# arclab-hku/ESVIO

Measured on AMD Instinct MI355X. Metric: Mevents/s through time-surface+detect+track @640x480, higher is better.
Workload: dtype f64 timestamps / u8 images / f32 LK sums in the reference build's order

## Files before the change

esvio_amd/csrc/fe_api.cpp:

```cpp
#include "fe_internal.h"

namespace {
typedef int (*nccl_allgather_fn)(const void*, void*, size_t, int , void* ,
                                 hipStream_t);
struct NcclId {
  char internal[128];
};
typedef int (*nccl_get_id_fn)(NcclId*);
typedef int (*nccl_init_rank_fn)(void** , int, NcclId, int);
typedef int (*nccl_destroy_fn)(void*);
void* rccl_lib() {
  static void* lib = []() -> void* {
    const char* names[] = {"librccl.so.1", "librccl.so"};
    for (const char* n : names)
      if (void* l = dlopen(n, RTLD_NOW | RTLD_NOLOAD | RTLD_GLOBAL)) return l;
    for (const char* n : names)
      if (void* l = dlopen(n, RTLD_NOW | RTLD_GLOBAL)) return l;
    return dlopen("/opt/rocm/lib/librccl.so.1", RTLD_NOW | RTLD_GLOBAL);
  }();
  return lib;
}
template <class F>
F rccl_sym(const char* name) {
  void* l = rccl_lib();
// ... 808 lines not shown
  }
  const auto t0 = std::chrono::steady_clock::now();
  while (tap.pending.load(std::memory_order_acquire) > 0 && std::chrono::steady_clock::now() - t0 < std::chrono::seconds(2)) {}
  host::ransac_pool_set_idle_work(pool, nullptr, nullptr, nullptr);
  out3[0] = tap.calls.load();
  out3[1] = tap.done.load();
  out3[2] = (uint64_t)std::max(0, tap.pending.load());
  host::ransac_pool_destroy(pool);
  if (n_inliers) *n_inliers = k;
  return 0;
}

int esvio_fe_lift_projective(const esvio_fe_camera* cam, double u, double v, double* out3) {
  if (!cam || !out3) return ESVIO_FE_EINVAL;
  host::lift_projective(*cam, u, v, out3);
  return 0;
}

static int fill_tracks(esvio_fe_handle c, esvio_fe_tracks* out);
static int track_event_entry(esvio_fe_handle c, double cur_time, const esvio_fe_event* left,
                             size_t nL, const esvio_fe_event* right, size_t nR, int space,
                             int pub_this_frame, const esvio_fe_motion* motion,
                             esvio_fe_tracks* out) {
  if (!c) return ESVIO_FE_EINVAL;
  if (nL == 0 || !left) return fail(c, ESVIO_FE_EINVAL, "left batch must not be empty (node:150)");
  if (nR && !right) return ESVIO_FE_EINVAL;
  if (nL + nR >= (1ull << 31)) return fail(c, ESVIO_FE_EINVAL, "batch too large");
  HIPCHK(c, hipSetDevice(c->dev));
  if (int rc = track_event_impl(c, cur_time, left, nL, right, nR, space, pub_this_frame != 0, motion))
    return rc;
// ... 3560 lines not shown
```

esvio_amd/csrc/fe_ctx.h:

```cpp
#pragma once
#include <hip/hip_runtime.h>

#include <algorithm>
#include <atomic>
#include <chrono>
#include <cmath>
#include <cstdarg>
#include <cstdio>
#include <cstdlib>
#include <cstring>
#include <dlfcn.h>
#include <map>
#include <string>
#include <utility>
#include <deque>
#include <vector>

#include "../../include/esvio_fe.h"
#include "../../include/esvio_fe_test.h"
#include "fe_aedat.h"
#include "fe_bag.h"
#include "fe_host.h"
#include "fe_kernels.h"
#include "fe_layout.h"
// ... 13 lines not shown
  void build(const std::vector<int>& ids, const std::vector<P2f>& pts) {
    v.clear();
    v.reserve(ids.size());
    for (size_t i = 0; i < ids.size(); i++) v.emplace_back(ids[i], pts[i]);
    std::stable_sort(v.begin(), v.end(),
                     [](const std::pair<int, P2f>& a, const std::pair<int, P2f>& b) { return a.first < b.first; });
    v.erase(std::unique(v.begin(), v.end(),
                        [](const std::pair<int, P2f>& a, const std::pair<int, P2f>& b) { return a.first == b.first; }),
            v.end());
  }
  const P2f* find(int id) const {
    auto it = std::lower_bound(v.begin(), v.end(), id,
                               [](const std::pair<int, P2f>& a, int k) { return a.first < k; });
    return (it != v.end() && it->first == id) ? &it->second : nullptr;
  }
};

const char* const kKernelNames[K_COUNT] = {
    "k_tile_hist", "k_tile_scan", "k_tile_scatter", "k_tile_apply", "k_sae_keys", "k_radix_pass", "k_sae_apply",
    "k_time_surface4", "k_time_surface", "k_median", "k_clahe", "k_norm_pyr", "k_pyr3", "k_pyr_down", "k_pyr_pad",
    "k_scharr", "k_pad_scharr", "k_lk_f32", "k_lk", "k_arc_map", "k_arc_ev", "k_dedup", "k_compact", "k_select_mw",
    "k_select", "k_select_gbm", "k_fast_score", "k_fast_collect", "k_events_from_fields", "k_baf_heads", "k_baf_filter",
    "k_baf_count", "k_baf_scan", "k_baf_emit", "k_baf_keys_fields", "k_baf_emit_fields", "k_raw_reduce", "k_raw_scan",
    "k_raw_emit", "k_slice_reduce", "k_slice_scan", "k_slice_cuts", "k_baf_keys_addr", "k_hot_count", "k_hot_keys",
    "k_hot_pick", "k_trig_reduce", "k_trig_emit"};
const char* const kIngestKernelNames[K_INGEST_COUNT - K_COUNT] = {"k_aedat_count", "k_aedat_scan", "k_aedat_emit", "k_bag_emit", "k_image_emit"};

enum Phase {
  PH_ENQ_BATCH, PH_ENQ_TEMPORAL, PH_WAIT_TEMPORAL, PH_FILTER, PH_RANSAC, PH_MASK_DETECT, PH_WAIT_STEREO, PH_TAIL,
  PH_PUB_SETMASK, PH_PUB_SELECT, PH_PUB_SPEC, PH_PUB_PREV_RIGHT, PH_PUB_STEREO_NEW, PH_PUB_PREFETCH,
// ... 446 lines not shown
    DevBuf<uint2> kids;
    DevBuf<int32_t> node_word;
    DevBuf<double> node_weight, word_weight;
    DevBuf<uint32_t> desc, keys[2], vals[2], sort, heads, q_word, cnt;
    DevBuf<int32_t> word, err;
    DevBuf<double> weight, q_val;
    uint32_t q_n = 0;
    DevBuf<uint32_t> db_word;
    DevBuf<double> db_val;
    DevBuf<uint64_t> db_off;
    std::vector<uint64_t> off = std::vector<uint64_t>(1, 0);
    DevBuf<double> score, res_score, res_raw;
    DevBuf<uint8_t> present;
    DevBuf<int32_t> res_id;
  } bow;
};

namespace esvio {
namespace fe {

inline thread_local hipStream_t t_stream_override = nullptr;
inline hipStream_t stereo_stream(const esvio_fe_ctx* c) { return c->stereo_unpub ? c->stream6 : c->stream4; }
inline hipStream_t cur_stream(const esvio_fe_ctx* c) {
  return t_stream_override ? t_stream_override : c->stream;
}
struct StreamScope {
  hipStream_t saved;
  explicit StreamScope(hipStream_t s) : saved(t_stream_override) { t_stream_override = s; }
  ~StreamScope() { t_stream_override = saved; }
};
// ... 96 lines not shown
```

esvio_amd/csrc/fe_host.cpp:

```cpp
#include "fe_host.h"

#include <algorithm>
#include <cfloat>
#include <climits>
#include <cmath>
#include <cstdio>
#include <cstdlib>
#include <cstring>

#include <atomic>
#include <chrono>
#include <condition_variable>
#include <sys/resource.h>
#include <memory>
#include <mutex>
#include <thread>

#if defined(__linux__)
#include <pthread.h>
#include <sched.h>
#endif

#if defined(__HIP_DEVICE_COMPILE__) || defined(ESVIO_NO_SIMD_CLONES)
#define ESVIO_SIMD_CLONES
#else
#define ESVIO_SIMD_CLONES __attribute__((target_clones("avx512f", "avx2", "default")))
#endif

namespace esvio {
namespace host {

int cv_round(double v) {
  if (!(v > -2147483648.5 && v < 2147483647.5)) return INT_MIN;
  const double r = std::nearbyint(v);
  if (r > 2147483647.0 || r < -2147483648.0) return INT_MIN;
  return (int)r;
}

int cv_floor(float v) {
  int i = (int)v;
  return i - (i > v);
}

static void radtan(const esvio_fe_camera& c, double x, double y, double& dx, double& dy) {
  const double x2 = x * x, y2 = y * y, xy = x * y;
  const double rho2 = x2 + y2;
  const double rad = c.k1 * rho2 + c.k2 * rho2 * rho2;
// ... 1353 lines not shown
```

esvio_amd/csrc/fe_host.h:

```cpp
#pragma once
#include <atomic>
#include <stdint.h>

#include <vector>

#include "../../include/esvio_fe.h"
#include "../../include/esvio_fe_test.h"

namespace esvio {
inline void cpu_relax() {
#if !defined(__HIP_DEVICE_COMPILE__) && (defined(__x86_64__) || defined(__i386__))
  __builtin_ia32_pause();
#endif
}
namespace host {

int cv_round(double v);
int cv_floor(float v);

void lift_projective(const esvio_fe_camera& cam, double u, double v, double out[3]);
void lift_projective_batch(const esvio_fe_camera& cam, const float* uv, int n, double* xu, double* yu);

std::vector<int> disc_halfwidths(int r);

struct BitMask {
  int W = 0, H = 0, wpr = 0;
  std::vector<uint32_t> bits;
  void reset(int w, int h);
  bool test(int x, int y) const { return (bits[(size_t)y * wpr + (x >> 5)] >> (x & 31)) & 1u; }
  void stamp_disc(int cx, int cy, int r, const std::vector<int>& hw);
  void from_bytes(const uint8_t* mask);
};
// ... 20 lines not shown
```

esvio_amd/csrc/fe_internal.h:

```cpp
#pragma once
#include "fe_ctx.h"

namespace esvio {
namespace fe {

template <class T>
void reduce_vector(std::vector<T>& v, const std::vector<uint8_t>& status) {
  int j = 0;
  for (int i = 0; i < int(v.size()); i++)
    if (status[i]) v[j++] = v[i];
  v.resize(j);
}

inline uint8_t* px00(const PyrDesc& d) { return d.img[0] + (size_t)kPad * d.stride[0] + kPad; }

inline int lookback_expired(esvio_fe_ctx* c) {
  return c->pin[0].counts[3] ? fail(c, ESVIO_FE_EINTERNAL, "radix sort look-back spin expired") : 0;
}

int ensure_event_capacity(esvio_fe_ctx* c, size_t n);
int ensure_sort_capacity(esvio_fe_ctx* c, size_t n);
int ensure_part_capacity(esvio_fe_ctx* c, size_t n, bool mc);
int ensure_cand_capacity(esvio_fe_ctx* c, int set, size_t n);
int ensure_arc_capacity(esvio_fe_ctx* c, size_t n, int set);
// ... 31 lines not shown
               int flags);
void run_lk(esvio_fe_ctx* c, const LkArgs& f, const LkArgs* b, float2* back_pts, uint8_t* back_status);
enum LkPairKind { kLkTemporal, kLkStereo };
struct LkPair {
  LkArgs f, b;
  LkOut out;
};
LkPair lk_pair(const PyrDesc& P, const PyrDesc& N, const P2f* src, const int* n_ptr, int n_max, LkPairKind kind,
               const LkOut& out);
void run_lk_pair(esvio_fe_ctx* c, const LkPair& p);
int copy_level0_out(esvio_fe_ctx* c, const PyrDesc& d, uint8_t* out);
int copy_level0_in(esvio_fe_ctx* c, const PyrDesc& d, const uint8_t* in, int space = ESVIO_FE_HOST);
bool in_border_event(const esvio_fe_ctx* c, const P2f& pt);
double pt_distance(const P2f& a, const P2f& b);
void event_set_mask(esvio_fe_ctx* c);
std::vector<P2f> undistorted_pts(const std::vector<P2f>& pts, const esvio_fe_camera& cam);
std::vector<P2f> pts_velocity_fn(std::vector<int>& ids, std::vector<P2f>& pts, IdMap& cur_id_pts,
                                 IdMap& prev_id_pts, double dt, size_t n_left);
void reject_with_f_event(esvio_fe_ctx* c);
void clear_tracker_state(esvio_fe_ctx* c);
SelectArgs make_select_args(esvio_fe_ctx* c, int set, int max_corners, float2* out_pts, int out_base,
                            int32_t* out_idx);
size_t select_lds_bytes(const esvio_fe_ctx* c);
KernelId launch_select_args(esvio_fe_ctx* c, SelectArgs s);
void compact_set(esvio_fe_ctx* c, const esvio_fe_ctx::CandSet& cs, uint32_t nblk, bool booked);
void run_select(esvio_fe_ctx* c, int set, int max_corners, float2* out_pts, int out_base, int32_t* out_idx,
                const uint32_t* mask_bits = nullptr, int* host_counts = nullptr, bool publish = false,
                const float2* stamp_pts = nullptr, int n_stamp = 0);
void run_arc(esvio_fe_ctx* c, const EventRec* ev, uint32_t n, const PyrDesc* ts, bool use_mask,
             bool want_flags, bool want_cand, int set, bool marked = false);
// ... 58 lines not shown
```

esvio_amd/csrc/fe_stages.cpp:

```cpp
#include "fe_internal.h"

#include <optional>

namespace esvio {
namespace fe {


int ensure_event_capacity(esvio_fe_ctx* c, size_t n) { return c->d_ev.grow(c, n); }

static int grow_sort_buffers(esvio_fe_ctx* c, size_t cap) {
  c->sort_cap = 0;
  for (int i = 0; i < 2; i++) {
    c->keys[i].release();
    c->vals[i].release();
  }
  for (int i = 0; i < 2; i++) {
    if (int rc = c->keys[i].alloc(c, cap)) return rc;
    if (int rc = c->vals[i].alloc(c, cap)) return rc;
  }
  if (int rc = c->sae_marks.alloc(c, cap)) return rc;
  c->sort_cap = cap;
  return 0;
}

// ... 481 lines not shown
}


bool in_border_event(const esvio_fe_ctx* c, const P2f& pt) {
  const int BORDER_SIZE = 1;
  const int img_x = host::cv_round(pt.x), img_y = host::cv_round(pt.y);
  return BORDER_SIZE <= img_x && img_x < c->W - BORDER_SIZE && BORDER_SIZE <= img_y &&
         img_y < c->H - BORDER_SIZE;
}

double pt_distance(const P2f& a, const P2f& b) {
  const double dx = a.x - b.x, dy = a.y - b.y;
  return std::sqrt(dx * dx + dy * dy);
}

void event_set_mask(esvio_fe_ctx* c) {
  c->mask_event.reset(c->W, c->H);
  struct Item {
    int first;
    std::pair<P2f, int> second;
    int src;
  };
  std::vector<Item> cnt_pts_id;
  cnt_pts_id.reserve(c->cur_pts.size());
  for (unsigned int i = 0; i < c->cur_pts.size(); i++)
    cnt_pts_id.push_back(Item{c->track_cnt[i], std::make_pair(c->cur_pts[i], c->ids[i]), c->src_idx[i]});
  std::sort(cnt_pts_id.begin(), cnt_pts_id.end(),
            [](const Item& a, const Item& b) { return a.first > b.first; });
  c->cur_pts.clear();
  c->ids.clear();
  c->track_cnt.clear();
  c->src_idx.clear();
  for (auto& it : cnt_pts_id) {
    const int px = host::cv_round(it.second.first.x), py = host::cv_round(it.second.first.y);
    if (px < 0 || px >= c->W || py < 0 || py >= c->H) continue;
    if (!c->mask_event.test(px, py)) {
      c->cur_pts.push_back(it.second.first);
      c->ids.push_back(it.second.second);
      c->track_cnt.push_back(it.first);
      c->src_idx.push_back(it.src);
      c->mask_event.stamp_disc(px, py, c->cfg.min_dist, c->hw);
    }
  }
}

std::vector<P2f> undistorted_pts(const std::vector<P2f>& pts, const esvio_fe_camera& cam) {
  const size_t n = pts.size();
  std::vector<P2f> un(n);
  if (!n) return un;
  std::vector<double> lx(n), ly(n);
  host::lift_projective_batch(cam, &pts[0].x, (int)n, lx.data(), ly.data());
  for (size_t i = 0; i < n; i++) un[i] = P2f{(float)lx[i], (float)ly[i]};
  return un;
}

std::vector<P2f> pts_velocity_fn(std::vector<int>& ids, std::vector<P2f>& pts, IdMap& cur_id_pts,
                                 IdMap& prev_id_pts, double dt, size_t n_left) {
  std::vector<P2f> vel;
// ... 10 lines not shown
        vel.push_back(P2f{0, 0});
      }
    }
  } else {
    vel.assign(n_left, P2f{0, 0});
  }
  return vel;
}

void reject_with_f_event(esvio_fe_ctx* c) {
  if (c->trace) c->tr_fm_class[c->cur_pts.size() < 8 ? 0 : c->cur_pts.size() < 15 ? 1 : 2]++;
  if (c->cur_pts.size() >= 8) {
    const esvio_fe_camera& cam = c->cfg.cam[0];
    const double FOCAL = c->cfg.focal_length;
    const size_t n = c->prev_pts.size();
    std::vector<float> un_cur(n * 2), un_prev(n * 2);
    std::vector<double> lx(n), ly(n);
    const double cx = c->W / 2.0, cy = c->H / 2.0;
    const auto tl = std::chrono::steady_clock::now();
    const bool pre = c->pre_lift_valid && c->pre_lx.size() == n;
    if (!pre) host::lift_projective_batch(cam, &c->prev_pts[0].x, (int)n, lx.data(), ly.data());
    const double* plx = pre ? c->pre_lx.data() : lx.data();
    const double* ply = pre ? c->pre_ly.data() : ly.data();
    c->pre_lift_valid = false;
    for (size_t i = 0; i < n; i++) {
      un_prev[2 * i] = (float)(FOCAL * plx[i] / 1.0 + cx);
      un_prev[2 * i + 1] = (float)(FOCAL * ply[i] / 1.0 + cy);
    }
    host::lift_projective_batch(cam, &c->cur_pts[0].x, (int)n, lx.data(), ly.data());
    for (size_t i = 0; i < n; i++) {
      un_cur[2 * i] = (float)(FOCAL * lx[i] / 1.0 + cx);
      un_cur[2 * i + 1] = (float)(FOCAL * ly[i] / 1.0 + cy);
    }
    std::vector<uint8_t> status(c->cur_pts.size());
    const auto t0 = std::chrono::steady_clock::now();
    host::find_fundamental_mat(un_prev.data(), un_cur.data(), (int)c->cur_pts.size(),
                               c->cfg.f_threshold, 0.99, status.data(), c->pool);
    if (c->trace) {
      const double ms = std::chrono::duration<double, std::milli>(std::chrono::steady_clock::now() - t0).count();
      c->tr_fm_ms += ms;
      c->tr_fm_max_ms = std::max(c->tr_fm_max_ms, ms);
      c->tr_lift_ms += std::chrono::duration<double, std::milli>(t0 - tl).count();
    }
    reduce_vector(c->prev_pts, status);
    reduce_vector(c->cur_pts, status);
    reduce_vector(c->ids, status);
    reduce_vector(c->track_cnt, status);
    reduce_vector(c->src_idx, status);
  }
// ... 166 lines not shown
```

esvio_amd/csrc/fe_track.cpp:

```cpp
#include "fe_internal.h"

#include <sched.h>
#include <sys/resource.h>

#include <atomic>
#include <condition_variable>
#include <mutex>
#include <thread>

namespace esvio {
namespace fe {

struct PrefetchJob {
  Inflight b;
  bool wait_planes = false;
  int lks_wait = -1;
};

static int prefetch_issue(esvio_fe_ctx* c, const PrefetchJob& j) {
  const Inflight& b = j.b;
  StreamScope on_prefetch_stream(c->stream2);
  PrefetchBatchScope its_event_images(&b);
  if (j.wait_planes) HIPCHK(c, hipStreamWaitEvent(c->stream2, c->ev_planes_free, 0));
  if (j.lks_wait >= 0) HIPCHK(c, hipStreamWaitEvent(c->stream2, c->ev_lks_done[j.lks_wait], 0));
  const EventRec *dL = b.dL, *dR = b.dR;
  if (b.stage >= 0) {
    if (int rc = stager_attach(c, b.stage, b.nL, c->stream2, &dL, &dR)) return rc;
  } else if (int rc = stage_events(c, b.left, b.nL, b.right, b.nR, b.space, &dL, &dR, b.lane)) {
    return rc;
  }
  bool arc_marked = false;
  McParams mcp;
// ... 46 lines not shown
        if ((++spins & 1023) == 0 &&
            std::chrono::steady_clock::now() - idle_since > std::chrono::microseconds(2000)) {
          std::unique_lock<std::mutex> lk(mu);
          sleeping.store(true, std::memory_order_seq_cst);
          cv.wait(lk, [&] {
            return submitted.load(std::memory_order_seq_cst) != done.load(std::memory_order_relaxed) ||
                   quit.load(std::memory_order_seq_cst);
          });
          sleeping.store(false, std::memory_order_seq_cst);
          idle_since = std::chrono::steady_clock::now();
        }
        continue;
      }
      const PrefetchJob& job = ring[d % kRing];
      if (first_rc.load(std::memory_order_relaxed) == 0) {
        const int rc = prefetch_issue(c, job);
        if (rc) first_rc.store(rc, std::memory_order_release);
      }
      if (first_rc.load(std::memory_order_relaxed) != 0 && job.b.gate) {
        launch_set_u32(c->stream2, c->d_lane_gate + job.b.lane, job.b.gate);
        (void)hipGetLastError();
      }
      done.store(d + 1, std::memory_order_release);
      idle_since = std::chrono::steady_clock::now();
    }
  }
};

int stereo_split_prepare(esvio_fe_ctx* c) {
  if (c->stream6) return 0;
  const bool wanted = c->stereo_split_env >= 0 ? c->stereo_split_env != 0 : (c->cfg.lk_accum == 2 && c->launcher != nullptr);
  if (!wanted) return 0;
  HIPCHK(c, c->stream6.create());
  launch_spin(c->stream6, 0);
  HIPCHK(c, hipStreamSynchronize(c->stream6));
  return 0;
}

int launcher_set(esvio_fe_ctx* c, bool on) {
  if (on == (c->launcher != nullptr)) return 0;
  if (on) {
    for (uint64_t& j : c->lane_job) j = 0;
    c->lks_wait_job[0] = c->lks_wait_job[1] = 0;
    Launcher* l = new Launcher();
    l->c = c;
    l->th = std::thread([l] { l->run(); });
    c->launcher = l;
    return 0;
  }
  const int rc = launcher_drain(c);
  if (rc && !c->launch_err) c->launch_err = rc;
  for (uint64_t& j : c->lane_job) j = 0;
  c->lks_wait_job[0] = c->lks_wait_job[1] = 0;
  Launcher* l = c->launcher;
  l->quit.store(true, std::memory_order_seq_cst);
  { std::lock_guard<std::mutex> g(l->mu); }
  l->cv.notify_all();
  l->th.join();
  delete l;
  c->launcher = nullptr;
  return rc;
}

static int launcher_result(esvio_fe_ctx* c) {
  const int rc = c->launcher->first_rc.load(std::memory_order_acquire);
  if (rc) c->err = c->launcher->err_text.empty() ? "a prefetch job of the launch thread failed" : c->launcher->err_text;
  return rc;
}

void launcher_clear_error(esvio_fe_ctx* c) {
  if (c->launcher) c->launcher->first_rc.store(0, std::memory_order_release);
  c->launch_err = 0;
}

int launcher_drain(esvio_fe_ctx* c) {
  Launcher* l = c->launcher;
  if (!l) return 0;
  while (l->done.load(std::memory_order_acquire) != l->submitted.load(std::memory_order_relaxed)) cpu_relax();
  return launcher_result(c);
}

int launcher_wait_lane(esvio_fe_ctx* c, int lane) {
  Launcher* l = c->launcher;
  if (!l) return 0;
  while (l->done.load(std::memory_order_acquire) < c->lane_job[lane]) cpu_relax();
  return launcher_result(c);
}

int record_lks_done(esvio_fe_ctx* c, int set) {
  if (Launcher* l = c->launcher) {
    while (l->done.load(std::memory_order_acquire) < c->lks_wait_job[set]) cpu_relax();
    if (int rc = launcher_result(c)) return rc;
  }
  HIPCHK(c, hipEventRecord(c->ev_lks_done[set], stereo_stream(c)));
  c->lks_last = set;
  return 0;
}

static int launcher_submit(esvio_fe_ctx* c, const PrefetchJob& j) {
  Launcher* l = c->launcher;
  const uint64_t s = l->submitted.load(std::memory_order_relaxed);
  l->ring[s % Launcher::kRing] = j;
  c->lane_job[j.b.lane] = s + 1;
  if (j.lks_wait >= 0) c->lks_wait_job[j.lks_wait] = s + 1;
  l->submitted.store(s + 1, std::memory_order_seq_cst);
  if (l->sleeping.load(std::memory_order_seq_cst)) {
    { std::lock_guard<std::mutex> g(l->mu); }
    l->cv.notify_all();
  }
  return 0;
}

int prefetch_next(esvio_fe_ctx* c, bool wait_planes, bool must_take_first) {
  int rc = 0;
  const bool only_first = must_take_first;
  const bool async_ok = c->launcher && !c->prof_on && !c->trace && !must_take_first;
  if (c->launcher && !async_ok)
    if ((rc = launcher_drain(c))) return rc;
  while (!rc && !c->announced.empty() && (int)c->inflight.size() < kPrefetchDepth) {
    PrefetchJob job;
    Inflight& b = job.b;
    static_cast<Batch&>(b) = c->announced.front();
    if (b.stage >= 0 && !must_take_first && !stager_ready(c, b.stage)) break;
    must_take_first = false;
// ... 92 lines not shown
  if (c->chain_enabled && c->waits_fit_chain && !nxt.pub && c->inflight.size() >= 2 && c->inflight[0].lane == nxt.lane &&
      !c->chain_valid)
    nxt2 = &c->inflight[1];
  if (nxt2) {
    sp.f.chain_out = c->d_chain;
    sp.f.chain_seq = next_chain_seq(c);
  }
  {
    StreamScope on_spec_stream(c->stream3);
    run_lk_pair(c, sp);
  }
  HIPCHK(c, hipEventRecord(c->ev_spec_done, c->stream3));
  c->spec_valid = true;
  if (nxt2) {
    const bool gated = c->launcher && nxt2->gate != 0;
    if (!gated)
      if (int rc = launcher_wait_lane(c, nxt2->lane)) return rc;
    HIPCHK(c, hipStreamWaitEvent(c->stream4, c->ev_lane_done[nxt.lane], 0));
    if (!gated) HIPCHK(c, hipStreamWaitEvent(c->stream4, c->ev_lane_done[nxt2->lane], 0));
    const PyrDesc& N2 = c->pyr[nxt2->slotL].d;
    LkPair ch = lk_pair(N, N2, nullptr, nullptr, n_max, kLkTemporal, c->zspec[1].out);
    ch.f.chain_in = c->d_chain;
    ch.f.chain_seq = c->chain_seq;
    ch.f.chain_ticks = c->lim.chain;
    ch.f.poll_err = c->zspec[1].expired;
    if (gated) {
      ch.f.gate_ptr = c->d_lane_gate + nxt2->lane;
      ch.f.gate_val = nxt2->gate;
    }
    {
// ... 2 lines not shown
    }
    HIPCHK(c, hipEventRecord(c->ev_chain_done, c->stream4));
    c->chain_valid = true;
    c->tr_chain_launch++;
    c->chain_for = c->frame_no + 2;
    c->chain_map_ok = false;
  }
  return 0;
}

int cancel_chain(esvio_fe_ctx* c) {
  if (!c->chain_valid) return 0;
  c->chain_valid = false;
  c->chain_map_ok = false;
  c->tr_chain_cancel++;
  HIPCHK(c, hipStreamSynchronize(c->stream4));
  return 0;
}

void right_tail(esvio_fe_ctx* c, const LkOut& kept, const P2f* left, const int* ids, const int* src,
                int n, int n_kept, double dt, size_t n_left) {
  const esvio_fe_config& cfg = c->cfg;
  c->ids_right.clear();
  c->cur_right_pts.clear();
  c->cur_un_right_pts.clear();
  c->right_pts_velocity.clear();
  c->cur_un_right_pts_map.clear();
  c->track_cnt_right.clear();
  if (n_left) {
    std::vector<uint8_t> status(n), statusRightLeft(n);
// ... 343 lines not shown
    c->pre_lift_valid = false;
    const PyrDesc& prevL = c->pyr[c->slot_prevL].d;
    const PyrDesc& curL = c->pyr[c->slot_curL].d;
    if (c->prev_pts.size() > 0) {
      const int n = (int)c->prev_pts.size();
      LkOut t{};
      bool spec_ok = false;
      if (use_spec) {
        if (int rc = await_early(c->ev_spec_done, 0, &spec_ok)) return rc;
        t = c->hspec[0].out;
        if (!spec_ok) {
          c->n_spec_expired++;
          HIPCHK(c, hipStreamSynchronize(c->stream3));
        }
      }
      std::vector<P2f> g_ptsB, g_ptsC;
      std::vector<uint8_t> g_stA, g_stB;
      if (use_chain) {
        if (int rc = await_early(c->ev_chain_done, 1, &spec_ok)) return rc;
        c->tr_chain_used += spec_ok;
        if (!spec_ok) c->n_chain_expired++;
        if (c->trace && spec_ok) trace_chain_intervals();
        if (spec_ok) {
          const LkOut& r = c->hspec[1].out;
          g_ptsB.resize(n);
          g_ptsC.resize(n);
          g_stA.resize(n);
          g_stB.resize(n);
          for (int j = 0; j < n; j++) {
            const int k = c->chain_map[j];
            g_ptsB[j] = r.fwd[k];
            g_ptsC[j] = r.back[k];
// ... 22 lines not shown
          st.f.chain_ticks = c->lim.chain;
          st.f.poll_err = c->zspec[1].expired;
          StreamScope on_stereo_stream(stereo_stream(c));
          HIPCHK(c, hipStreamWaitEvent(stereo_stream(c), c->ev_imgs_ready, 0));
          run_lk_pair(c, st);
          if (int rc = record_lks_done(c, c->res_set)) return rc;
        }
        if (int rc = early_work()) return rc;
        if (int rc = exchange_flush(c)) return rc;
        pre_lift();
        lap(PH_ENQ_TEMPORAL);
        HIPCHK(c, sync_main(c));
        lap(PH_WAIT_TEMPORAL);
        t = pin.s1;
      }
      std::vector<uint8_t> status(t.st_fwd, t.st_fwd + n);
      c->cur_pts.resize(n);
      std::memcpy(c->cur_pts.data(), t.fwd, (size_t)n * 8);
      if (cfg.flow_back) {
        const P2f* reverse_pts = t.back;
        for (int i = 0; i < n; i++) {
          if (status[i] && t.st_back[i] && pt_distance(c->prev_pts[i], reverse_pts[i]) <= 0.5)
            status[i] = 1;
          else
            status[i] = 0;
        }
      }
      for (int i = 0; i < n; i++)
        if (status[i] && !in_border_event(c, c->cur_pts[i])) status[i] = 0;
      if (chain_covers_next) {
        if (use_spec && spec_ok) {
// ... 59 lines not shown
    const PyrDesc& curR = c->pyr[c->slot_curR].d;
    n_surv = (int)c->cur_pts.size();
    c->src_idx.resize(n_surv);
    for (int i = 0; i < n_surv; i++) c->src_idx[i] = stereo_chained ? surv_src[i] : i;
    lap(PH_FILTER);
    n_kept = n_surv;
    will_spec = (have_next || had_announced) && c->waits_fit_spec;
    if (!PUB_THIS_FRAME) {
      if (int rc = upload_kept()) return rc;
      if (will_spec && n_kept && !c->chain_valid)
        if (const Inflight* nb = next_batch())
          if (int rc = enqueue_spec_temporal(c, *nb, n_kept, false)) return rc;
    }
    if (n_surv && !stereo_chained) {
      std::memcpy(pin.A, c->cur_pts.data(), (size_t)n_surv * 8);
      {
        StreamScope on_stereo_stream(stereo_stream(c));
        run_lk_pair(c, lk_pair(curL, curR, zpin.A, nullptr, n_surv, kLkStereo, zpin.s1));
        if (int rc = record_lks_done(c, c->res_set)) return rc;
      }
    }
    return 0;
  }

  int publish() {
    const esvio_fe_config& cfg = c->cfg;
    const PyrDesc& curL = c->pyr[c->slot_curL].d;
    const PyrDesc& curR = c->pyr[c->slot_curR].d;
    if (PUB_THIS_FRAME) {
      if (cfg.f_ransac) reject_with_f_event(c);
      lap(PH_RANSAC);
      PhaseClock parts;
      auto sub = [&](Phase p) { c->lat.cur_phase[p] += parts.lap(); };
// ... 61 lines not shown
        c->cur_pts.push_back(p);
        c->ids.push_back(c->n_id++);
        c->track_cnt.push_back(1);
      }
    }
    const int pub = PUB_THIS_FRAME ? 1 : 0;
    PhaseClock tt;
    auto tail_lap = [&](int i) { if (c->trace) c->tail_ms[pub][i] += tt.lap(); };
    c->cur_un_pts = undistorted_pts(c->cur_pts, cfg.cam[0]);
    c->pts_velocity = pts_velocity_fn(c->ids, c->cur_un_pts, c->cur_un_pts_map, c->prev_un_pts_map,
                                      c->cur_time - c->prev_time, c->cur_pts.size());
    lap(PH_TAIL);
    tail_lap(0);
    const bool lazy = c->lazy_new && detect;
    const bool defer_right = c->lazy_new && !PUB_THIS_FRAME;
    bool pending_later = false;
    if (defer_right && c->pend.active && !c->pend_right.active) {
      pending_later = c->lazy_late || !event_over(c->ev_lknew_done);
    }
    if (!pending_later)
      if (int rc = finalize_lazy(c)) return rc;
    tail_lap(1);
    if (defer_right) {
    } else {
      if (!lazy) HIPCHK(c, sync_main(c));
      if (n_surv || stereo_chained) HIPCHK(c, sync_event(c->ev_lks_done[c->res_set]));
      if (stereo_chained) {
        if (take_expired(1)) {
          c->n_chain_expired++;
          const int n = (int)surv_src.size() ? surv_src.back() + 1 : 0;
          if (n) {
            const PyrDesc& curL = c->pyr[c->slot_curL].d;
            const PyrDesc& curR = c->pyr[c->slot_curR].d;
            StreamScope on_stereo_stream(stereo_stream(c));
            run_lk_pair(c, lk_pair(curL, curR, zpin.s1.fwd, nullptr, n, kLkStereo, c->zpin[set_st].s1));
            HIPCHK(c, hipStreamSynchronize(stereo_stream(c)));
          }
        }
      }
    }
// ... 120 lines not shown
  c->stereo_unpub = !PUB_THIS_FRAME && c->stereo_split;
  c->frame_no++;
  t.pin = c->pin[c->res_set];
  t.zpin = c->zpin[c->res_set];
  if (PUB_THIS_FRAME && c->pool) host::ransac_pool_wake(c->pool);
  c->cur_time = _cur_time;
  c->lat.cur_phase[PH_CHECK] = t.clock.lap();
  int rc = t.take_batch();
  if (!rc) {
    t.lap(PH_ENQ_BATCH);
    rc = t.temporal();
  }
  if (!rc) rc = t.survivors_stereo();
  if (!rc) rc = t.publish();
  if (!rc) rc = t.tails();
  if (rc && c->cur_stage >= 0) {
    (void)launcher_drain(c);
    (void)hipStreamSynchronize(c->stream);
    (void)hipStreamSynchronize(c->stream2);
    (void)hipStreamSynchronize(c->stream4);
    if (c->stream6) (void)hipStreamSynchronize(c->stream6);
    (void)hipGetLastError();
    stager_abandon(c, c->cur_stage);
    c->cur_stage = -1;
  }
  if (!rc) latency_commit(c, PUB_THIS_FRAME, t0, cpu0, sw0, allocs0);
  return rc;
}


// ... 3 lines not shown
```

esvio_amd/frontend.py:

```python
import ctypes as C
import os

import numpy as np

from . import build as _build

_HERE = os.path.dirname(os.path.abspath(__file__))
HOST, DEVICE = 0, 1
EVENT_IMAGES_AHEAD = 2
LK_USE_INITIAL_FLOW = 4


class FrontendError(RuntimeError):
    pass


class Camera(C.Structure):
    _fields_ = [(n, C.c_double) for n in ("fx", "fy", "cx", "cy", "k1", "k2", "p1", "p2")]


class Config(C.Structure):
    _fields_ = [
        ("width", C.c_int32), ("height", C.c_int32),
        ("decay_ms", C.c_double),
# ... 282 lines not shown
    "esvio_fe_track_image", "esvio_fe_unregister_host_buffer", "esvio_fe_version",
    "esvio_fe_kf_set_pattern", "esvio_fe_kf_blur", "esvio_fe_kf_fast", "esvio_fe_kf_brief", "esvio_fe_kf_match",
    "esvio_fe_kf_describe",
    "esvio_fe_bow_vocabulary_header", "esvio_fe_bow_set_vocabulary", "esvio_fe_bow_transform", "esvio_fe_bow_add",
    "esvio_fe_bow_query", "esvio_fe_bow_detect_loop", "esvio_fe_bow_clear", "esvio_fe_bow_entries", "esvio_fe_bow_reserve",
]
TEST_SYMBOLS = [
    "esvio_fe_build_pyramid", "esvio_fe_debug_counters", "esvio_fe_debug_inject", "esvio_fe_device_memory",
    "esvio_fe_export_level",
    "esvio_fe_find_fundamental_mat_held", "esvio_fe_find_fundamental_mat_idle", "esvio_fe_find_fundamental_mat_mt",
    "esvio_fe_get_kernel_stats", "esvio_fe_host_hypot", "esvio_fe_host_nullspace", "esvio_fe_host_stage_copy",
    "esvio_fe_host_stage_pack", "esvio_fe_staging_counters",
    "esvio_fe_kernel_count", "esvio_fe_kernel_name", "esvio_fe_latency_phase_name", "esvio_fe_latency_recent",
    "esvio_fe_latency_stats", "esvio_fe_lift_projective", "esvio_fe_plain_call_counters", "esvio_fe_ransac_stats",
    "esvio_fe_ransac_tail", "esvio_fe_raw_tile_bytes", "esvio_fe_reset_kernel_stats", "esvio_fe_select_candidates",
    "esvio_fe_set_profiling", "esvio_fe_set_sae",
    "esvio_fe_slice_tile_events", "esvio_fe_stage_kernel_count", "esvio_fe_stream",
    "esvio_fe_aedat_tile_events", "esvio_fe_ingest_kernel_count", "esvio_fe_aedat_walk_tap", "esvio_fe_aedat_walk_state_bytes",
    "esvio_fe_bag_tile_events", "esvio_fe_bag_walk_tap", "esvio_fe_bag_walk_state_bytes",
    "esvio_fe_bag_image_walk_tap", "esvio_fe_image_tile_pixels", "esvio_fe_event_image_kernel_stats",
    "esvio_fe_aedat_frame_walk_tap", "esvio_fe_aedat_frame_kernel_stats", "esvio_fe_frame16_tile_pixels",
    "esvio_fe_kf_kernel_count", "esvio_fe_kf_kernel_name", "esvio_fe_kf_kernel_stats", "esvio_fe_kf_blur_tile",
    "esvio_fe_bow_kernel_count", "esvio_fe_bow_kernel_name", "esvio_fe_bow_kernel_stats", "esvio_fe_bow_limits", "esvio_fe_bow_scores",
]

LATENCY_PHASES = 16
SELECT_EUCLID, SELECT_TABLE = 1, 2


class LatencyCall(C.Structure):
    _fields_ = [("call", C.c_uint64), ("published", C.c_int32), ("reserved", C.c_int32), ("begin_ms", C.c_double),
# ... 1763 lines not shown
    rc = L.esvio_fe_lift_projective(C.byref(c), float(u), float(v), _p(out))
    if rc:
        raise FrontendError("lift_projective rc=%d" % rc)
    return out


def aedat_header(data):
    buf = bytes(data)
    info = AedatHeaderInfo()
    rc = load_library().esvio_fe_aedat_header(buf if buf else None, len(buf), C.byref(info))
    if rc:
        raise FrontendError("esvio_fe_aedat_header rc=%d" % rc)
    return info


def aedat_walk_tap(state, data, runs_cap=None, events_cap=None):
    L = load_library()
    nst = L.esvio_fe_aedat_walk_state_bytes()
    st = np.zeros(nst, np.uint8) if state is None else np.frombuffer(bytes(state), np.uint8).copy()
    buf = np.frombuffer(bytes(data), np.uint8)
    events_cap = buf.nbytes // 8 + 1 if events_cap is None else events_cap
    runs_cap = events_cap if runs_cap is None else runs_cap
    runs, pay, counts = np.zeros((max(runs_cap, 1), 2), np.uint32), np.zeros(max(events_cap, 1) * 8, np.uint8), np.zeros(4, np.uint64)
    rc = L.esvio_fe_aedat_walk_tap(_p(st), nst, _p(buf) if buf.nbytes else None, buf.nbytes, _p(runs), runs_cap, _p(pay), events_cap, _p(counts))
    if rc:
        raise FrontendError("esvio_fe_aedat_walk_tap rc=%d" % rc)
    n, nr = int(counts[0]), int(counts[1])
    r = np.stack([runs[:nr, 0].astype(np.int64), runs[:nr, 1].view(np.int32).astype(np.int64)], axis=1) if nr else np.zeros((0, 2), np.int64)
    return st.tobytes(), r, pay[:8 * n].tobytes(), tuple(int(v) for v in counts)

# ... 77 lines not shown
```

Measured before the change: 2943.

## Cut host overhead: SIMD set_mask, inline cvRound, scratch reuse, async stereo LK launch

Replaces the bitmap-stamping set_mask with a pairwise check against kept points, using SSE2 to reject candidates eight at a time, and makes cv_round an inline SSE2 conversion. Per-frame vectors in reject/filter are moved into reusable context scratch to avoid allocations. The stereo LK launch is handed to the launcher thread on publish frames, with waits added before dependent syncs. It also drops a pending-later event check and adds a test tap; these add synchronization complexity and could change rounding or behavior in edge cases.

```diff
diff --git a/esvio_amd/csrc/fe_api.cpp b/esvio_amd/csrc/fe_api.cpp
--- a/esvio_amd/csrc/fe_api.cpp
+++ b/esvio_amd/csrc/fe_api.cpp
@@ -846,6 +846,35 @@
 int esvio_fe_lift_projective(const esvio_fe_camera* cam, double u, double v, double* out3) {
   if (!cam || !out3) return ESVIO_FE_EINVAL;
   host::lift_projective(*cam, u, v, out3);
+  return 0;
+}
+
+int esvio_fe_set_mask_tap(int width, int height, int min_dist, int form, const float* xy, const int32_t* ids,
+                          const int32_t* track_cnt, int n, float* out_xy, int32_t* out_ids, int32_t* out_cnt,
+                          int32_t* out_src, int32_t* n_out) {
+  if (width <= 0 || height <= 0 || min_dist < 1 || min_dist > kMaxDiscR || (form != 0 && form != 1) || n < 0 || !n_out)
+    return ESVIO_FE_EINVAL;
+  if (n && (!xy || !ids || !track_cnt || !out_xy || !out_ids || !out_cnt || !out_src)) return ESVIO_FE_EINVAL;
+  std::vector<P2f> pts(n);
+  std::vector<int> id(n), cnt(n), src(n);
+  for (int i = 0; i < n; i++) {
+    pts[i] = P2f{xy[2 * i], xy[2 * i + 1]};
+    id[i] = ids[i];
+    cnt[i] = track_cnt[i];
+    src[i] = i;
+  }
+  SetMaskScratch scratch;
+  host::BitMask bitmap;
+  set_mask_points(width, height, min_dist, host::disc_halfwidths(min_dist), pts, id, cnt, src, scratch,
+                  form ? &bitmap : nullptr);
+  for (size_t k = 0; k < pts.size(); k++) {
+    out_xy[2 * k] = pts[k].x;
+    out_xy[2 * k + 1] = pts[k].y;
+    out_ids[k] = id[k];
+    out_cnt[k] = cnt[k];
+    out_src[k] = src[k];
+  }
+  *n_out = (int32_t)pts.size();
   return 0;
 }
 
diff --git a/esvio_amd/csrc/fe_ctx.h b/esvio_amd/csrc/fe_ctx.h
--- a/esvio_amd/csrc/fe_ctx.h
+++ b/esvio_amd/csrc/fe_ctx.h
@@ -51,6 +51,21 @@
                                [](const std::pair<int, P2f>& a, int k) { return a.first < k; });
     return (it != v.end() && it->first == id) ? &it->second : nullptr;
   }
+};
+
+struct SetMaskItem {
+  int first;
+  std::pair<P2f, int> second;
+  int src;
+};
+struct SetMaskScratch {
+  std::vector<SetMaskItem> items;
+  std::vector<int16_t> kx, ky;
+};
+struct RejectScratch {
+  std::vector<float> un_cur, un_prev;
+  std::vector<double> lx, ly;
+  std::vector<uint8_t> status;
 };
 
 const char* const kKernelNames[K_COUNT] = {
@@ -527,6 +542,14 @@
     DevBuf<uint8_t> present;
     DevBuf<int32_t> res_id;
   } bow;
+
+  SetMaskScratch set_mask_scratch;
+  RejectScratch reject_scratch;
+  struct FilterScratch {
+    std::vector<uint8_t> status, stA, stB;
+    std::vector<P2f> ptsB, ptsC;
+  } filter_scratch;
+  uint64_t stereo_job = 0;
 };
 
 namespace esvio {
diff --git a/esvio_amd/csrc/fe_host.cpp b/esvio_amd/csrc/fe_host.cpp
--- a/esvio_amd/csrc/fe_host.cpp
+++ b/esvio_amd/csrc/fe_host.cpp
@@ -30,7 +30,7 @@
 namespace esvio {
 namespace host {
 
-int cv_round(double v) {
+int cv_round_portable(double v) {
   if (!(v > -2147483648.5 && v < 2147483647.5)) return INT_MIN;
   const double r = std::nearbyint(v);
   if (r > 2147483647.0 || r < -2147483648.0) return INT_MIN;
diff --git a/esvio_amd/csrc/fe_host.h b/esvio_amd/csrc/fe_host.h
--- a/esvio_amd/csrc/fe_host.h
+++ b/esvio_amd/csrc/fe_host.h
@@ -7,6 +7,11 @@
 #include "../../include/esvio_fe.h"
 #include "../../include/esvio_fe_test.h"
 
+#if !defined(__HIP_DEVICE_COMPILE__) && defined(__x86_64__)
+#include <emmintrin.h>
+#define ESVIO_HOST_SSE2 1
+#endif
+
 namespace esvio {
 inline void cpu_relax() {
 #if !defined(__HIP_DEVICE_COMPILE__) && (defined(__x86_64__) || defined(__i386__))
@@ -15,7 +20,14 @@
 }
 namespace host {
 
-int cv_round(double v);
+int cv_round_portable(double v);
+inline int cv_round(double v) {
+#ifdef ESVIO_HOST_SSE2
+  return _mm_cvtsd_si32(_mm_set_sd(v));
+#else
+  return cv_round_portable(v);
+#endif
+}
 int cv_floor(float v);
 
 void lift_projective(const esvio_fe_camera& cam, double u, double v, double out[3]);
diff --git a/esvio_amd/csrc/fe_internal.h b/esvio_amd/csrc/fe_internal.h
--- a/esvio_amd/csrc/fe_internal.h
+++ b/esvio_amd/csrc/fe_internal.h
@@ -69,6 +69,8 @@
 bool in_border_event(const esvio_fe_ctx* c, const P2f& pt);
 double pt_distance(const P2f& a, const P2f& b);
 void event_set_mask(esvio_fe_ctx* c);
+void set_mask_points(int W, int H, int r, const std::vector<int>& hw, std::vector<P2f>& pts, std::vector<int>& ids,
+                     std::vector<int>& track_cnt, std::vector<int>& src_idx, SetMaskScratch& s, host::BitMask* bitmap);
 std::vector<P2f> undistorted_pts(const std::vector<P2f>& pts, const esvio_fe_camera& cam);
 std::vector<P2f> pts_velocity_fn(std::vector<int>& ids, std::vector<P2f>& pts, IdMap& cur_id_pts,
                                  IdMap& prev_id_pts, double dt, size_t n_left);
diff --git a/esvio_amd/csrc/fe_stages.cpp b/esvio_amd/csrc/fe_stages.cpp
--- a/esvio_amd/csrc/fe_stages.cpp
+++ b/esvio_amd/csrc/fe_stages.cpp
@@ -1,6 +1,11 @@
 #include "fe_internal.h"
 
 #include <optional>
+
+#if !defined(__HIP_DEVICE_COMPILE__) && defined(__x86_64__)
+#include <emmintrin.h>
+#define ESVIO_SET_MASK_SSE2 1
+#endif
 
 namespace esvio {
 namespace fe {
@@ -519,34 +524,76 @@
   return std::sqrt(dx * dx + dy * dy);
 }
 
-void event_set_mask(esvio_fe_ctx* c) {
-  c->mask_event.reset(c->W, c->H);
-  struct Item {
-    int first;
-    std::pair<P2f, int> second;
-    int src;
+static bool in_kept_disc(const int16_t* kx, const int16_t* ky, int nk, int px, int py, int r, const int* hw) {
+  auto exact = [&](int j) {
+    const int dy = std::abs(py - ky[j]), dx = std::abs(px - kx[j]);
+    return dy <= r && dx <= hw[dy];
   };
-  std::vector<Item> cnt_pts_id;
-  cnt_pts_id.reserve(c->cur_pts.size());
-  for (unsigned int i = 0; i < c->cur_pts.size(); i++)
-    cnt_pts_id.push_back(Item{c->track_cnt[i], std::make_pair(c->cur_pts[i], c->ids[i]), c->src_idx[i]});
+  int j = 0;
+#ifdef ESVIO_SET_MASK_SSE2
+  const __m128i vx = _mm_set1_epi16((short)(px + r)), vy = _mm_set1_epi16((short)(py + r));
+  const __m128i lim = _mm_set1_epi16((short)(2 * r)), zero = _mm_setzero_si128();
+  for (; j + 8 <= nk; j += 8) {
+    const __m128i ex = _mm_subs_epu16(_mm_sub_epi16(vx, _mm_loadu_si128((const __m128i*)(kx + j))), lim);
+    const __m128i ey = _mm_subs_epu16(_mm_sub_epi16(vy, _mm_loadu_si128((const __m128i*)(ky + j))), lim);
+    int m = _mm_movemask_epi8(_mm_cmpeq_epi16(_mm_or_si128(ex, ey), zero));
+    for (; m; m &= m - 1) {
+      const int bit = __builtin_ctz((unsigned)m);
+      if (!(bit & 1) && exact(j + (bit >> 1))) return true;
+    }
+  }
+#endif
+  for (; j < nk; j++)
+    if (exact(j)) return true;
+  return false;
+}
+
+void set_mask_points(int W, int H, int r, const std::vector<int>& hw, std::vector<P2f>& pts, std::vector<int>& ids,
+                     std::vector<int>& track_cnt, std::vector<int>& src_idx, SetMaskScratch& s, host::BitMask* bitmap) {
+  if (bitmap) bitmap->reset(W, H);
+  using Item = SetMaskItem;
+  std::vector<Item>& cnt_pts_id = s.items;
+  cnt_pts_id.clear();
+  cnt_pts_id.reserve(pts.size());
+  for (unsigned int i = 0; i < pts.size(); i++)
+    cnt_pts_id.push_back(Item{track_cnt[i], std::make_pair(pts[i], ids[i]), src_idx[i]});
   std::sort(cnt_pts_id.begin(), cnt_pts_id.end(),
             [](const Item& a, const Item& b) { return a.first > b.first; });
-  c->cur_pts.clear();
-  c->ids.clear();
-  c->track_cnt.clear();
-  c->src_idx.clear();
+  pts.clear();
+  ids.clear();
+  track_cnt.clear();
+  src_idx.clear();
+  s.kx.resize(cnt_pts_id.size());
+  s.ky.resize(cnt_pts_id.size());
+  int nk = 0;
+  const bool pairwise = !bitmap && W <= 16384 && H <= 16384 && r <= 255;
+  host::BitMask own;
+  if (!bitmap && !pairwise) {
+    own.reset(W, H);
+    bitmap = &own;
+  }
   for (auto& it : cnt_pts_id) {
     const int px = host::cv_round(it.second.first.x), py = host::cv_round(it.second.first.y);
-    if (px < 0 || px >= c->W || py < 0 || py >= c->H) continue;
-    if (!c->mask_event.test(px, py)) {
-      c->cur_pts.push_back(it.second.first);
-      c->ids.push_back(it.second.second);
-      c->track_cnt.push_back(it.first);
-      c->src_idx.push_back(it.src);
-      c->mask_event.stamp_disc(px, py, c->cfg.min_dist, c->hw);
+    if (px < 0 || px >= W || py < 0 || py >= H) continue;
+    if (bitmap ? !bitmap->test(px, py) : !in_kept_disc(s.kx.data(), s.ky.data(), nk, px, py, r, hw.data())) {
+      pts.push_back(it.second.first);
+      ids.push_back(it.second.second);
+      track_cnt.push_back(it.first);
+      src_idx.push_back(it.src);
+      if (bitmap) {
+        bitmap->stamp_disc(px, py, r, hw);
+      } else {
+        s.kx[nk] = (int16_t)px;
+        s.ky[nk] = (int16_t)py;
+        nk++;
+      }
     }
   }
+}
+
+void event_set_mask(esvio_fe_ctx* c) {
+  set_mask_points(c->W, c->H, c->cfg.min_dist, c->hw, c->cur_pts, c->ids, c->track_cnt, c->src_idx, c->set_mask_scratch,
+                  nullptr);
 }
 
 std::vector<P2f> undistorted_pts(const std::vector<P2f>& pts, const esvio_fe_camera& cam) {
@@ -587,8 +634,13 @@
     const esvio_fe_camera& cam = c->cfg.cam[0];
     const double FOCAL = c->cfg.focal_length;
     const size_t n = c->prev_pts.size();
-    std::vector<float> un_cur(n * 2), un_prev(n * 2);
-    std::vector<double> lx(n), ly(n);
+    RejectScratch& s = c->reject_scratch;
+    std::vector<float>&un_cur = s.un_cur, &un_prev = s.un_prev;
+    std::vector<double>&lx = s.lx, &ly = s.ly;
+    un_cur.resize(n * 2);
+    un_prev.resize(n * 2);
+    lx.resize(n);
+    ly.resize(n);
     const double cx = c->W / 2.0, cy = c->H / 2.0;
     const auto tl = std::chrono::steady_clock::now();
     const bool pre = c->pre_lift_valid && c->pre_lx.size() == n;
@@ -605,7 +657,8 @@
       un_cur[2 * i] = (float)(FOCAL * lx[i] / 1.0 + cx);
       un_cur[2 * i + 1] = (float)(FOCAL * ly[i] / 1.0 + cy);
     }
-    std::vector<uint8_t> status(c->cur_pts.size());
+    std::vector<uint8_t>& status = s.status;
+    status.assign(c->cur_pts.size(), 0);
     const auto t0 = std::chrono::steady_clock::now();
     host::find_fundamental_mat(un_prev.data(), un_cur.data(), (int)c->cur_pts.size(),
                                c->cfg.f_threshold, 0.99, status.data(), c->pool);
diff --git a/esvio_amd/csrc/fe_track.cpp b/esvio_amd/csrc/fe_track.cpp
--- a/esvio_amd/csrc/fe_track.cpp
+++ b/esvio_amd/csrc/fe_track.cpp
@@ -15,7 +15,18 @@
   Inflight b;
   bool wait_planes = false;
   int lks_wait = -1;
+  bool stereo = false;
+  LkPair lk{};
+  hipStream_t stream = nullptr;
+  int lks_set = 0;
 };
+
+static int stereo_issue(esvio_fe_ctx* c, const PrefetchJob& j) {
+  StreamScope on_stereo_stream(j.stream);
+  run_lk_pair(c, j.lk);
+  HIPCHK(c, hipEventRecord(c->ev_lks_done[j.lks_set], j.stream));
+  return 0;
+}
 
 static int prefetch_issue(esvio_fe_ctx* c, const PrefetchJob& j) {
   const Inflight& b = j.b;
@@ -92,7 +103,7 @@
       }
       const PrefetchJob& job = ring[d % kRing];
       if (first_rc.load(std::memory_order_relaxed) == 0) {
-        const int rc = prefetch_issue(c, job);
+        const int rc = job.stereo ? stereo_issue(c, job) : prefetch_issue(c, job);
         if (rc) first_rc.store(rc, std::memory_order_release);
       }
       if (first_rc.load(std::memory_order_relaxed) != 0 && job.b.gate) {
@@ -120,6 +131,7 @@
   if (on) {
     for (uint64_t& j : c->lane_job) j = 0;
     c->lks_wait_job[0] = c->lks_wait_job[1] = 0;
+    c->stereo_job = 0;
     Launcher* l = new Launcher();
     l->c = c;
     l->th = std::thread([l] { l->run(); });
@@ -130,6 +142,7 @@
   if (rc && !c->launch_err) c->launch_err = rc;
   for (uint64_t& j : c->lane_job) j = 0;
   c->lks_wait_job[0] = c->lks_wait_job[1] = 0;
+  c->stereo_job = 0;
   Launcher* l = c->launcher;
   l->quit.store(true, std::memory_order_seq_cst);
   { std::lock_guard<std::mutex> g(l->mu); }
@@ -158,6 +171,15 @@
   return launcher_result(c);
 }
 
+static int launcher_wait_stereo(esvio_fe_ctx* c) {
+  if (!c->stereo_job) return 0;
+  const uint64_t job = std::exchange(c->stereo_job, 0);
+  Launcher* l = c->launcher;
+  if (!l) return 0;
+  while (l->done.load(std::memory_order_acquire) < job) cpu_relax();
+  return launcher_result(c);
+}
+
 int launcher_wait_lane(esvio_fe_ctx* c, int lane) {
   Launcher* l = c->launcher;
   if (!l) return 0;
@@ -166,6 +188,7 @@
 }
 
 int record_lks_done(esvio_fe_ctx* c, int set) {
+  if (int rc = launcher_wait_stereo(c)) return rc;
   if (Launcher* l = c->launcher) {
     while (l->done.load(std::memory_order_acquire) < c->lks_wait_job[set]) cpu_relax();
     if (int rc = launcher_result(c)) return rc;
@@ -173,6 +196,14 @@
   HIPCHK(c, hipEventRecord(c->ev_lks_done[set], stereo_stream(c)));
   c->lks_last = set;
   return 0;
+}
+
+static void launcher_publish(Launcher* l, uint64_t s) {
+  l->submitted.store(s + 1, std::memory_order_seq_cst);
+  if (l->sleeping.load(std::memory_order_seq_cst)) {
+    { std::lock_guard<std::mutex> g(l->mu); }
+    l->cv.notify_all();
+  }
 }
 
 static int launcher_submit(esvio_fe_ctx* c, const PrefetchJob& j) {
@@ -181,11 +212,23 @@
   l->ring[s % Launcher::kRing] = j;
   c->lane_job[j.b.lane] = s + 1;
   if (j.lks_wait >= 0) c->lks_wait_job[j.lks_wait] = s + 1;
-  l->submitted.store(s + 1, std::memory_order_seq_cst);
-  if (l->sleeping.load(std::memory_order_seq_cst)) {
-    { std::lock_guard<std::mutex> g(l->mu); }
-    l->cv.notify_all();
-  }
+  launcher_publish(l, s);
+  return 0;
+}
+
+static int launcher_submit_stereo(esvio_fe_ctx* c, const LkPair& lk, hipStream_t stream, int set) {
+  if (int rc = launcher_wait_stereo(c)) return rc;
+  Launcher* l = c->launcher;
+  const uint64_t s = l->submitted.load(std::memory_order_relaxed);
+  PrefetchJob& j = l->ring[s % Launcher::kRing];
+  j.stereo = true;
+  j.b.gate = 0;
+  j.lk = lk;
+  j.stream = stream;
+  j.lks_set = set;
+  c->stereo_job = s + 1;
+  c->lks_last = set;
+  launcher_publish(l, s);
   return 0;
 }
 
@@ -308,6 +351,7 @@
   c->spec_valid = true;
   if (nxt2) {
     const bool gated = c->launcher && nxt2->gate != 0;
+    if (int rc = launcher_wait_stereo(c)) return rc;
     if (!gated)
       if (int rc = launcher_wait_lane(c, nxt2->lane)) return rc;
     HIPCHK(c, hipStreamWaitEvent(c->stream4, c->ev_lane_done[nxt.lane], 0));
@@ -340,6 +384,7 @@
   c->chain_valid = false;
   c->chain_map_ok = false;
   c->tr_chain_cancel++;
+  if (int rc = launcher_wait_stereo(c)) return rc;
   HIPCHK(c, hipStreamSynchronize(c->stream4));
   return 0;
 }
@@ -713,8 +758,8 @@
           HIPCHK(c, hipStreamSynchronize(c->stream3));
         }
       }
-      std::vector<P2f> g_ptsB, g_ptsC;
-      std::vector<uint8_t> g_stA, g_stB;
+      std::vector<P2f>&g_ptsB = c->filter_scratch.ptsB, &g_ptsC = c->filter_scratch.ptsC;
+      std::vector<uint8_t>&g_stA = c->filter_scratch.stA, &g_stB = c->filter_scratch.stB;
       if (use_chain) {
         if (int rc = await_early(c->ev_chain_done, 1, &spec_ok)) return rc;
         c->tr_chain_used += spec_ok;
@@ -767,7 +812,8 @@
         lap(PH_WAIT_TEMPORAL);
         t = pin.s1;
       }
-      std::vector<uint8_t> status(t.st_fwd, t.st_fwd + n);
+      std::vector<uint8_t>& status = c->filter_scratch.status;
+      status.assign(t.st_fwd, t.st_fwd + n);
       c->cur_pts.resize(n);
       std::memcpy(c->cur_pts.data(), t.fwd, (size_t)n * 8);
       if (cfg.flow_back) {
@@ -857,9 +903,12 @@
     }
     if (n_surv && !stereo_chained) {
       std::memcpy(pin.A, c->cur_pts.data(), (size_t)n_surv * 8);
-      {
+      const LkPair st = lk_pair(curL, curR, zpin.A, nullptr, n_surv, kLkStereo, zpin.s1);
+      if (PUB_THIS_FRAME && c->launcher && !c->prof_on && !c->trace) {
+        if (int rc = launcher_submit_stereo(c, st, stereo_stream(c), c->res_set)) return rc;
+      } else {
         StreamScope on_stereo_stream(stereo_stream(c));
-        run_lk_pair(c, lk_pair(curL, curR, zpin.A, nullptr, n_surv, kLkStereo, zpin.s1));
+        run_lk_pair(c, st);
         if (int rc = record_lks_done(c, c->res_set)) return rc;
       }
     }
@@ -951,16 +1000,14 @@
     tail_lap(0);
     const bool lazy = c->lazy_new && detect;
     const bool defer_right = c->lazy_new && !PUB_THIS_FRAME;
-    bool pending_later = false;
-    if (defer_right && c->pend.active && !c->pend_right.active) {
-      pending_later = c->lazy_late || !event_over(c->ev_lknew_done);
-    }
+    const bool pending_later = defer_right && c->pend.active && !c->pend_right.active;
     if (!pending_later)
       if (int rc = finalize_lazy(c)) return rc;
     tail_lap(1);
     if (defer_right) {
     } else {
       if (!lazy) HIPCHK(c, sync_main(c));
+      if (int rc = launcher_wait_stereo(c)) return rc;
       if (n_surv || stereo_chained) HIPCHK(c, sync_event(c->ev_lks_done[c->res_set]));
       if (stereo_chained) {
         if (take_expired(1)) {
@@ -1111,6 +1158,8 @@
   if (!rc) rc = t.survivors_stereo();
   if (!rc) rc = t.publish();
   if (!rc) rc = t.tails();
+  if (int rc2 = launcher_wait_stereo(c))
+    if (!rc) rc = rc2;
   if (rc && c->cur_stage >= 0) {
     (void)launcher_drain(c);
     (void)hipStreamSynchronize(c->stream);
diff --git a/esvio_amd/frontend.py b/esvio_amd/frontend.py
--- a/esvio_amd/frontend.py
+++ b/esvio_amd/frontend.py
@@ -320,7 +320,7 @@
     "esvio_fe_kernel_count", "esvio_fe_kernel_name", "esvio_fe_latency_phase_name", "esvio_fe_latency_recent",
     "esvio_fe_latency_stats", "esvio_fe_lift_projective", "esvio_fe_plain_call_counters", "esvio_fe_ransac_stats",
     "esvio_fe_ransac_tail", "esvio_fe_raw_tile_bytes", "esvio_fe_reset_kernel_stats", "esvio_fe_select_candidates",
-    "esvio_fe_set_profiling", "esvio_fe_set_sae",
+    "esvio_fe_set_mask_tap", "esvio_fe_set_profiling", "esvio_fe_set_sae",
     "esvio_fe_slice_tile_events", "esvio_fe_stage_kernel_count", "esvio_fe_stream",
     "esvio_fe_aedat_tile_events", "esvio_fe_ingest_kernel_count", "esvio_fe_aedat_walk_tap", "esvio_fe_aedat_walk_state_bytes",
     "esvio_fe_bag_tile_events", "esvio_fe_bag_walk_tap", "esvio_fe_bag_walk_state_bytes",
@@ -2114,6 +2114,25 @@
     return info
 
 
+def set_mask_tap(width, height, min_dist, xy, ids, track_cnt, form=0):
+    L = load_library()
+    xy = np.ascontiguousarray(xy, np.float32).reshape(-1, 2)
+    ids = np.ascontiguousarray(ids, np.int32)
+    cnt = np.ascontiguousarray(track_cnt, np.int32)
+    n = len(ids)
+    assert len(xy) == n and len(cnt) == n
+    oxy, oid, ocnt, osrc = np.zeros((max(n, 1), 2), np.float32), np.zeros(max(n, 1), np.int32), np.zeros(max(n, 1), np.int32), np.zeros(max(n, 1), np.int32)
+    k = C.c_int32()
+    L.esvio_fe_set_mask_tap.restype = C.c_int
+    rc = L.esvio_fe_set_mask_tap(C.c_int(int(width)), C.c_int(int(height)), C.c_int(int(min_dist)), C.c_int(int(form)),
+                                 _p(xy) if n else None, _p(ids) if n else None, _p(cnt) if n else None, C.c_int(n),
+                                 _p(oxy), _p(oid), _p(ocnt), _p(osrc), C.byref(k))
+    if rc:
+        raise FrontendError("esvio_fe_set_mask_tap rc=%d" % rc)
+    k = k.value
+    return oxy[:k].copy(), oid[:k].copy(), ocnt[:k].copy(), osrc[:k].copy()
+
+
 def aedat_walk_tap(state, data, runs_cap=None, events_cap=None):
     L = load_library()
     nst = L.esvio_fe_aedat_walk_state_bytes()
```

After: 3069 (median of 6 runs). +4.3%, better.
